# sungnyun/dualhyp

Hardware: AMD Instinct MI355X
Metric: corrected utterances/sec (TinyLlama-1.1B, 5+5 hyps, 512->64 tok) (higher is better)
Workload: dtype bf16; 1 GPU; DualHyp inference, TinyLlama-1.1B bf16 + LoRA r16 (q,k,v,proj), batch 32/GPU synthetic 5+5-hyp prompts, 512-token prompt -> 64 generated tokens, greedy; batch_per_gpu=32, parallelism=replicas x1, batches_in_flight_per_gpu=64, schedule=merged, decode_rows_per_launch=2048

## Files before the change

dualhyp_amd/csrc/capi.hip:

```cpp
#include "common.h"
#include "tuning.h"
#include <stdarg.h>

static thread_local char g_err[512] = "";

void dh_set_error(const char* fmt, ...) {
    va_list ap;
    va_start(ap, fmt);
    vsnprintf(g_err, sizeof(g_err), fmt, ap);
    va_end(ap);
}

extern "C" const char* dh_last_error(void) { return g_err; }
extern "C" int dh_abi_version(void) { return DH_ABI_VERSION; }

extern "C" int dh_device_info(char* h_buf, int h_buf_len, int* h_num_cu, int64_t* h_hbm_bytes) {
    int n = 0;
    hipError_t e = hipGetDeviceCount(&n);
    DH_CHECK(e == hipSuccess && n > 0, "no HIP device visible (%s)", hipGetErrorString(e));
    int dev = 0;
    DH_HIP(hipGetDevice(&dev));
    hipDeviceProp_t p;
    DH_HIP(hipGetDeviceProperties(&p, dev));
    if (h_buf && h_buf_len > 0) {
        strncpy(h_buf, p.gcnArchName, h_buf_len - 1);
        h_buf[h_buf_len - 1] = 0;
    }
    if (h_num_cu) *h_num_cu = p.multiProcessorCount;
    if (h_hbm_bytes) *h_hbm_bytes = (int64_t)p.totalGlobalMem;
    return 0;
}

namespace {

enum Accept { ANY, BOOL , RANGE , ONE_OF  };
struct TuningRow { int key; int* knob; Accept accept; int a, b, c; };
constexpr int NO_MAX = 0x7fffffff;

const TuningRow TUNING[] = {
    {0, &g_skinny_variant, ANY, 0, 0, 0},
    {1, &g_gemm_variant, ANY, 0, 0, 0},
    {2, &g_swiglu2, ANY, 0, 0, 0},
    {3, &g_mid, ANY, 0, 0, 0},
    {4, &g_linear_phase, ANY, 0, 0, 0},
    {5, &g_gemm_gm, RANGE, 0, NO_MAX, 0},
    {6, &g_dt_min_rows, RANGE, 1, NO_MAX, 0},
    {7, &g_chain_min_rows, RANGE, 1, NO_MAX, 0},
    {8, &g_dt_stages, ANY, 0, 0, 0},
    {9, &g_gemm128_stages, ANY, 0, 0, 0},
    {10, &g_decode_tiled_rows, RANGE, 0, NO_MAX, 0},
    {11, &g_rows_ct, RANGE, 0, NO_MAX, 0},
    {12, &g_fuse_qkv_rope, ANY, 0, 0, 0},
    {13, &g_mid_wlds, ANY, 0, 0, 0},
    {14, &g_rows_ng, ONE_OF, 0, 8, 10},
    {15, &g_dt_wide, ANY, 0, 0, 0},
    {16, &g_short_kps, ONE_OF, 8, 16, 16},
    {17, &g_pairs_wn, ONE_OF, 0, 2, 4},
    {18, &g_pairs_min_rows, RANGE, 1, NO_MAX, 0},
    {19, &g_fp8_tile, ONE_OF, 0, 128, 256},
    {20, &g_fp8_gm, RANGE, 0, 64, 0},
    {21, &g_pairs_wt, BOOL, 0, 0, 0},
    {22, &g_w4_persist, RANGE, 0, 2, 0},
    {23, &g_prune_last_layer, BOOL, 0, 0, 0},
    {24, &g_w4_fast_epi, ANY, 0, 0, 0},
    {25, &g_w4_persist_qkv, BOOL, 0, 0, 0},
    {26, &g_tn_mfma, BOOL, 0, 0, 0},
    {27, &g_attn_bwd_dq_group, BOOL, 0, 0, 0},
    {28, &g_tail_split, BOOL, 0, 0, 0},
    {29, &g_attn_bwd_dkdv_img, BOOL, 0, 0, 0},
    {30, &g_w4_persist_lora, BOOL, 0, 0, 0},
    {31, &g_skinny_n, BOOL, 0, 0, 0},
};

}

extern "C" int dh_set_tuning(int key, int value) {
    for (const TuningRow& r : TUNING) {
        if (r.key != key) continue;
        if (r.accept == RANGE && (value < r.a || value > r.b)) break;
        if (r.accept == ONE_OF && value != r.a && value != r.b && value != r.c) break;
        *r.knob = r.accept == BOOL ? value != 0 : value;
        return 0;
    }
    dh_set_error("dh_set_tuning: unknown key %d", key);
    return 1;
}
```

dualhyp_amd/csrc/decode_fused.hip:

```cpp
#include "common.h"

namespace {

constexpr int DCOLS = 16;
constexpr int MAXP = 16;

template <int HS, int PMAX, int NW>
__global__ __launch_bounds__(NW * 64, NW == 16 ? 1 : (NW == 6 ? 3 : (HS == 64 ? 4 : 2))) void attn_decode_fused_kernel(
    const float* __restrict__ qkv32, int n_part, int pairs, int n_seq, int ldq, int qkv_dim,
    const bf16_t* __restrict__ lora_b, float lora_scale, int split0, int split1,
    const bf16_t* __restrict__ cos, const bf16_t* __restrict__ sin, const int32_t* __restrict__ seq_slot,
    const int32_t* __restrict__ kv_len, bf16_t* __restrict__ k_cache, bf16_t* __restrict__ vT_cache,
    bf16_t* __restrict__ y, int n_head, int n_groups, int s_max, float scale) {
    constexpr int KS = HS / 16, DT = HS / 32, HALF = HS / 2;
    extern __shared__ __attribute__((aligned(16))) char smem[];
    const int pair = blockIdx.x, seq = pair / n_groups, g = pair % n_groups;
    const int q_per_kv = n_head / n_groups;
    const int tid = threadIdx.x, lane = tid & 63, wave = tid >> 6;
    const int lr = lane & 31, lh = lane >> 5;
    const int slot = seq_slot[seq];
    const int len = kv_len[seq], pos = len - 1;
    bf16_t* sQ = reinterpret_cast<bf16_t*>(smem);
    float* sKn = reinterpret_cast<float*>(smem + 16 * HS * 2);
    float* sVn = sKn + HS;
    float* sXa = sVn + HS;
    float* sSn = sXa + 48;
    float* sPm = sSn + 16;
    float* sPl = sPm + NW * DCOLS;
    float* sPo = sPl + NW * DCOLS;
    constexpr int NT_ = NW * 64;

    constexpr int PF = NW == 6 ? 2 : 1;
    struct VF { bf16x8 v; };
    struct Tile { bf16x8 kf[KS]; VF vf[DT][2]; };
    Tile tl[PF];
    const bf16_t* kbase = k_cache + ((size_t)slot * n_groups + g) * s_max * HS;
    const bf16_t* vbase = vT_cache + ((size_t)slot * n_groups + g) * HS * s_max;
    const int n_tiles = (pos + 31) / 32;
    auto load_tile = [&](Tile& T, int t) {
#pragma unroll
        for (int ks = 0; ks < KS; ++ks)
            T.kf[ks] = __builtin_nontemporal_load(reinterpret_cast<const bf16x8*>(kbase + kfrag_blk<HS>(t, ks) + lane * 8));
#pragma unroll
        for (int dt = 0; dt < DT; ++dt)
#pragma unroll
            for (int s2 = 0; s2 < 2; ++s2)
                T.vf[dt][s2].v = __builtin_nontemporal_load(reinterpret_cast<const bf16x8*>(vbase + vfrag_blk<HS>(t, dt, s2) + lane * 8));
    };
#pragma unroll
    for (int p = 0; p < PF; ++p)
        if (wave + NW * p < n_tiles) load_tile(tl[p], wave + NW * p);

    const float* row0 = qkv32 + (size_t)seq * ldq;
    const size_t pstride = (size_t)n_seq * ldq;
    auto psum = [&](int c) {
        float v[PMAX];
#pragma unroll
        for (int p = 0; p < PMAX; ++p) v[p] = p < n_part ? row0[p * pstride + c] : 0.f;
        float s = 0.f;
        if (pairs) {
#pragma unroll
            for (int p = 0; p < PMAX; p += 2) s += v[p] + v[p + 1];
        } else {
#pragma unroll
            for (int p = 0; p < PMAX; ++p) s += v[p];
        }
        return s;
    };
    if (lora_b != nullptr && tid < 48) sXa[tid] = rbf(psum(qkv_dim + tid));
    for (int i = tid; i < 16 * HS; i += NT_) sQ[i] = 0;
    __syncthreads();

    auto finish = [&](int c) -> float {
        float o = rbf(psum(c));
        if (lora_b != nullptr) {
            const int seg = (c >= split0) + (c >= split1);
            const uint4* b4 = reinterpret_cast<const uint4*>(lora_b + (size_t)c * 16);
            float l = 0.f;
#pragma unroll
            for (int h = 0; h < 2; ++h) {
                const uint4 bv = b4[h];
                const bf16_t* bp = reinterpret_cast<const bf16_t*>(&bv);
#pragma unroll
                for (int e = 0; e < 8; ++e) l = fmaf(sXa[seg * 16 + h * 8 + e], bf2f(bp[e]), l);
            }
            o = rbf(o + rbf(rbf(l) * lora_scale));
        }
        return o;
    };
    const int gbase = g * (q_per_kv + 2) * HS;
    bf16_t* kdst = k_cache + ((size_t)slot * n_groups + g) * s_max * HS;
    bf16_t* vdst = vT_cache + ((size_t)slot * n_groups + g) * HS * s_max;
    const int n_rope = (q_per_kv + 1) * HALF;
    for (int it = tid; it < n_rope + HS; it += NT_) {
        if (it < n_rope) {
            const int j = it / HALF, i = it % HALF;
            const float x1 = finish(gbase + j * HS + i), x2 = finish(gbase + j * HS + HALF + i);
            const bf16_t* cp = cos + (size_t)pos * HS;
            const bf16_t* sp = sin + (size_t)pos * HS;
            const bf16_t o1 = f2bf(rbf(x1 * bf2f(cp[i])) + rbf(-x2 * bf2f(sp[i])));
            const bf16_t o2 = f2bf(rbf(x2 * bf2f(cp[HALF + i])) + rbf(x1 * bf2f(sp[HALF + i])));
            if (j < q_per_kv) {
                sQ[j * HS + i] = o1;
                sQ[j * HS + HALF + i] = o2;
            } else {
                sKn[i] = bf2f(o1);
                sKn[HALF + i] = bf2f(o2);
                kdst[kfrag_off<HS>(pos, i)] = o1;
                kdst[kfrag_off<HS>(pos, HALF + i)] = o2;
            }
        } else {
            const int e = it - n_rope;
            const bf16_t v = f2bf(finish(gbase + (q_per_kv + 1) * HS + e));
            sVn[e] = bf2f(v);
            vdst[vfrag_off<HS>(pos, e)] = v;
        }
    }
    __syncthreads();

    for (int h = wave; h < q_per_kv; h += NW) {
        float p = 0.f;
        for (int e = lane; e < HS; e += 64) p += bf2f(sQ[h * HS + e]) * sKn[e];
        p = wave_sum(p);
        if (lane == 0) sSn[h] = p * scale;
    }

    bf16x8 qf[KS];
#pragma unroll
    for (int ks = 0; ks < KS; ++ks) qf[ks] = *reinterpret_cast<const bf16x8*>(sQ + (lr & 15) * HS + ks * 16 + lh * 8);
    if (lr >= 16) {
#pragma unroll
        for (int ks = 0; ks < KS; ++ks) qf[ks] = bf16x8{0, 0, 0, 0, 0, 0, 0, 0};
    }
    f32x16 o[DT];
#pragma unroll
    for (int dt = 0; dt < DT; ++dt)
#pragma unroll
        for (int r = 0; r < 16; ++r) o[dt][r] = 0.f;
    float m_run = -INFINITY, l_run = 0.f;
    auto compute_tile = [&](const Tile& T, int t) {
        const int key0 = t * 32;
        f32x16 st;
#pragma unroll
        for (int r = 0; r < 16; ++r) st[r] = 0.f;
#pragma unroll
        for (int ks = 0; ks < KS; ++ks) st = __builtin_amdgcn_mfma_f32_32x32x16_bf16(T.kf[ks], qf[ks], st, 0, 0, 0);
        float m_t = -INFINITY;
#pragma unroll
        for (int r = 0; r < 16; ++r) {
            const int key_abs = key0 + (r & 3) + 8 * (r >> 2) + 4 * lh;
            float sc = st[r] * scale;
            sc = key_abs < pos ? sc : -INFINITY;
            st[r] = sc;
            m_t = fmaxf(m_t, sc);
        }
        m_t = fmaxf(m_t, __shfl_xor(m_t, 32, 64));
        const float m_new = fmaxf(m_run, m_t);
        const float alpha = __expf(m_run - m_new);
        m_run = m_new;
        float psm = 0.f;
#pragma unroll
        for (int r = 0; r < 16; ++r) {
            const float p = __expf(st[r] - m_new);
            st[r] = p;
            psm += p;
        }
        l_run = l_run * alpha + psm;
#pragma unroll
        for (int s2 = 0; s2 < 2; ++s2) {
            union { bf16x8 v; uint32_t u[4]; } pf;
#pragma unroll
            for (int j = 0; j < 4; ++j) pf.u[j] = pack2bf(st[8 * s2 + 2 * j], st[8 * s2 + 2 * j + 1]);
#pragma unroll
            for (int dt = 0; dt < DT; ++dt) {
                if (s2 == 0) {
#pragma unroll
                    for (int r = 0; r < 16; ++r) o[dt][r] *= alpha;
                }
                o[dt] = __builtin_amdgcn_mfma_f32_32x32x16_bf16(T.vf[dt][s2].v, pf.v, o[dt], 0, 0, 0);
            }
        }
    };
    for (int base = wave; base < n_tiles; base += NW * PF) {
#pragma unroll
        for (int p = 0; p < PF; ++p) {
            if (base + NW * p < n_tiles) compute_tile(tl[p], base + NW * p);
            if (base + NW * (PF + p) < n_tiles) load_tile(tl[p], base + NW * (PF + p));
        }
    }
    const float l_tot = l_run + __shfl_xor(l_run, 32, 64);
    if (lr < q_per_kv) {
        if (lh == 0) {
            sPm[wave * DCOLS + lr] = m_run;
            sPl[wave * DCOLS + lr] = l_tot;
        }
#pragma unroll
        for (int dt = 0; dt < DT; ++dt)
#pragma unroll
            for (int r = 0; r < 16; ++r) {
                const int d = dt * 32 + (r & 3) + 8 * (r >> 2) + 4 * lh;
                sPo[(wave * HS + d) * DCOLS + lr] = o[dt][r];
            }
    }
    __syncthreads();
    for (int it = tid; it < q_per_kv * HS; it += NT_) {
        const int h = it / HS, d = it % HS;
        const float sn = sSn[h];
        float M = sn;
#pragma unroll
        for (int w = 0; w < NW; ++w) M = fmaxf(M, sPm[w * DCOLS + h]);
        const float pn = __expf(sn - M);
        float L = pn, O = rbf(pn) * sVn[d];
#pragma unroll
        for (int w = 0; w < NW; ++w) {
            const float mw = sPm[w * DCOLS + h];
            const float f = (mw == -INFINITY) ? 0.f : __expf(mw - M);
            L += sPl[w * DCOLS + h] * f;
            O += sPo[(w * HS + d) * DCOLS + h] * f;
        }
        y[(size_t)seq * n_head * HS + (g * q_per_kv + h) * HS + d] = f2bf(O / L);
    }
}

#ifndef DH_ATTN_WAVES64
#define DH_ATTN_WAVES64 8
#endif
template <int HS>
constexpr int attn_fused_waves() { return HS == 64 ? DH_ATTN_WAVES64 : 8; }
template <int HS>
constexpr size_t attn_fused_lds() {
    constexpr int NW = attn_fused_waves<HS>();
    return 16 * HS * 2 + (HS + HS + 48 + 16 + NW * DCOLS + NW * DCOLS + NW * HS * DCOLS) * sizeof(float);
}

template <int HS, int PMAX, int NW>
__global__ __launch_bounds__(NW * 64, 1) void attn_verify_fused_kernel(
    const float* __restrict__ qkv32, int n_part, int pairs, int n_rows, int ldq, int qkv_dim,
    const bf16_t* __restrict__ lora_b, float lora_scale, int split0, int split1,
    const bf16_t* __restrict__ cos, const bf16_t* __restrict__ sin, const int32_t* __restrict__ seq_slot,
    const int32_t* __restrict__ kv_len, bf16_t* __restrict__ k_cache, bf16_t* __restrict__ vT_cache,
    bf16_t* __restrict__ y, int n_head, int n_groups, int s_max, int p_max, int S, float scale) {
    constexpr int KS = HS / 16, DT = HS / 32, HALF = HS / 2, VC = 32;
    extern __shared__ __attribute__((aligned(16))) char smem[];
    const int pair = blockIdx.x, seq = pair / n_groups, g = pair % n_groups;
    const int q_per_kv = n_head / n_groups, ncol = S * q_per_kv;
    const int tid = threadIdx.x, lane = tid & 63, wave = tid >> 6;
    const int lr = lane & 31, lh = lane >> 5;
    const int slot = seq_slot[seq];
    const int len = kv_len[seq], pos = len - 1;
    const int n_live = min(S, p_max - pos);
    bf16_t* sQ = reinterpret_cast<bf16_t*>(smem);
    float* sKn = reinterpret_cast<float*>(smem + VC * HS * 2);
    float* sVn = sKn + S * HS;
    float* sXa = sVn + S * HS;
    float* sSn = sXa + S * 48;
    float* sPm = sSn + VC;
    float* sPl = sPm + NW * VC;
    float* sPo = sPl + NW * VC;
    constexpr int NT_ = NW * 64;

    struct VF { bf16x8 v; };
    struct Tile { bf16x8 kf[KS]; VF vf[DT][2]; };
    Tile tl;
    const bf16_t* kbase = k_cache + ((size_t)slot * n_groups + g) * s_max * HS;
    const bf16_t* vbase = vT_cache + ((size_t)slot * n_groups + g) * HS * s_max;
    const int n_tiles = (pos + n_live - 1 + 31) / 32;
    const int t_safe = pos >> 5;
    auto load_tile = [&](Tile& T, int t, bool early) {
#pragma unroll
        for (int ks = 0; ks < KS; ++ks) {
            const bf16x8* p = reinterpret_cast<const bf16x8*>(kbase + kfrag_blk<HS>(t, ks) + lane * 8);
            T.kf[ks] = early ? __builtin_nontemporal_load(p) : *p;
        }
#pragma unroll
        for (int dt = 0; dt < DT; ++dt)
#pragma unroll
            for (int s2 = 0; s2 < 2; ++s2) {
                const bf16x8* p = reinterpret_cast<const bf16x8*>(vbase + vfrag_blk<HS>(t, dt, s2) + lane * 8);
                T.vf[dt][s2].v = early ? __builtin_nontemporal_load(p) : *p;
            }
    };
    if (wave < t_safe) load_tile(tl, wave, true);

    const size_t pstride = (size_t)n_rows * ldq;
    auto psum = [&](int j, int c) {
        const float* row0 = qkv32 + ((size_t)seq * S + j) * ldq;
        float v[PMAX];
#pragma unroll
        for (int p = 0; p < PMAX; ++p) v[p] = p < n_part ? row0[p * pstride + c] : 0.f;
        float s = 0.f;
        if (pairs) {
#pragma unroll
            for (int p = 0; p < PMAX; p += 2) s += v[p] + v[p + 1];
        } else {
#pragma unroll
            for (int p = 0; p < PMAX; ++p) s += v[p];
        }
        return s;
    };
    if (lora_b != nullptr)
        for (int i = tid; i < 48 * S; i += NT_) sXa[i] = rbf(psum(i / 48, qkv_dim + i % 48));
    for (int i = tid; i < VC * HS; i += NT_) sQ[i] = 0;
    for (int i = tid; i < 2 * S * HS; i += NT_) sKn[i] = 0.f;
    __syncthreads();

    auto finish = [&](int j, int c) -> float {
        float o = rbf(psum(j, c));
        if (lora_b != nullptr) {
            const int seg = (c >= split0) + (c >= split1);
            const uint4* b4 = reinterpret_cast<const uint4*>(lora_b + (size_t)c * 16);
            float l = 0.f;
#pragma unroll
            for (int h = 0; h < 2; ++h) {
                const uint4 bv = b4[h];
                const bf16_t* bp = reinterpret_cast<const bf16_t*>(&bv);
#pragma unroll
                for (int e = 0; e < 8; ++e) l = fmaf(sXa[j * 48 + seg * 16 + h * 8 + e], bf2f(bp[e]), l);
            }
            o = rbf(o + rbf(rbf(l) * lora_scale));
        }
        return o;
    };
    const int gbase = g * (q_per_kv + 2) * HS;
    bf16_t* kdst = k_cache + ((size_t)slot * n_groups + g) * s_max * HS;
    bf16_t* vdst = vT_cache + ((size_t)slot * n_groups + g) * HS * s_max;
    const int n_rope = (q_per_kv + 1) * HALF, per_row = n_rope + HS;
    for (int it0 = tid; it0 < n_live * per_row; it0 += NT_) {
        const int jr = it0 / per_row, it = it0 % per_row, pj = pos + jr;
        if (it < n_rope) {
            const int j = it / HALF, i = it % HALF;
            const float x1 = finish(jr, gbase + j * HS + i), x2 = finish(jr, gbase + j * HS + HALF + i);
            const bf16_t* cp = cos + (size_t)pj * HS;
            const bf16_t* sp = sin + (size_t)pj * HS;
            const bf16_t o1 = f2bf(rbf(x1 * bf2f(cp[i])) + rbf(-x2 * bf2f(sp[i])));
            const bf16_t o2 = f2bf(rbf(x2 * bf2f(cp[HALF + i])) + rbf(x1 * bf2f(sp[HALF + i])));
            if (j < q_per_kv) {
                sQ[(jr * q_per_kv + j) * HS + i] = o1;
                sQ[(jr * q_per_kv + j) * HS + HALF + i] = o2;
            } else {
                sKn[jr * HS + i] = bf2f(o1);
                sKn[jr * HS + HALF + i] = bf2f(o2);
                kdst[kfrag_off<HS>(pj, i)] = o1;
                kdst[kfrag_off<HS>(pj, HALF + i)] = o2;
            }
        } else {
            const int e = it - n_rope;
            const bf16_t v = f2bf(finish(jr, gbase + (q_per_kv + 1) * HS + e));
            sVn[jr * HS + e] = bf2f(v);
            vdst[vfrag_off<HS>(pj, e)] = v;
        }
    }
    __threadfence_block();
    __syncthreads();
    if (wave >= t_safe && wave < n_tiles) load_tile(tl, wave, false);

    for (int c = wave; c < ncol; c += NW) {
        const float* kn = sKn + (c / q_per_kv) * HS;
        float p = 0.f;
        for (int e = lane; e < HS; e += 64) p += bf2f(sQ[c * HS + e]) * kn[e];
        p = wave_sum(p);
        if (lane == 0) sSn[c] = p * scale;
    }

    bf16x8 qf[KS];
#pragma unroll
    for (int ks = 0; ks < KS; ++ks) qf[ks] = *reinterpret_cast<const bf16x8*>(sQ + lr * HS + ks * 16 + lh * 8);
    const int j_col = lr < ncol ? lr / q_per_kv : 0;
    const int p_col = pos + (j_col < n_live ? j_col : 0);
    f32x16 o[DT];
#pragma unroll
    for (int dt = 0; dt < DT; ++dt)
#pragma unroll
        for (int r = 0; r < 16; ++r) o[dt][r] = 0.f;
    float m_run = -INFINITY, l_run = 0.f;
    auto compute_tile = [&](const Tile& T, int t) {
        const int key0 = t * 32;
        f32x16 st;
#pragma unroll
        for (int r = 0; r < 16; ++r) st[r] = 0.f;
#pragma unroll
        for (int ks = 0; ks < KS; ++ks) st = __builtin_amdgcn_mfma_f32_32x32x16_bf16(T.kf[ks], qf[ks], st, 0, 0, 0);
        float m_t = -INFINITY;
#pragma unroll
        for (int r = 0; r < 16; ++r) {
            const int key_abs = key0 + (r & 3) + 8 * (r >> 2) + 4 * lh;
            float sc = st[r] * scale;
            sc = key_abs < p_col ? sc : -INFINITY;
            st[r] = sc;
            m_t = fmaxf(m_t, sc);
        }
        m_t = fmaxf(m_t, __shfl_xor(m_t, 32, 64));
        const float m_new = fmaxf(m_run, m_t);
        const bool none = m_new == -INFINITY;
        const float alpha = none ? 1.f : __expf(m_run - m_new);
        m_run = m_new;
        float psm = 0.f;
#pragma unroll
        for (int r = 0; r < 16; ++r) {
            const float p = none ? 0.f : __expf(st[r] - m_new);
            st[r] = p;
            psm += p;
        }
        l_run = l_run * alpha + psm;
#pragma unroll
        for (int s2 = 0; s2 < 2; ++s2) {
            union { bf16x8 v; uint32_t u[4]; } pf;
#pragma unroll
            for (int j = 0; j < 4; ++j) pf.u[j] = pack2bf(st[8 * s2 + 2 * j], st[8 * s2 + 2 * j + 1]);
#pragma unroll
            for (int dt = 0; dt < DT; ++dt) {
                if (s2 == 0) {
#pragma unroll
                    for (int r = 0; r < 16; ++r) o[dt][r] *= alpha;
                }
                o[dt] = __builtin_amdgcn_mfma_f32_32x32x16_bf16(T.vf[dt][s2].v, pf.v, o[dt], 0, 0, 0);
            }
        }
    };
    for (int base = wave; base < n_tiles; base += NW) {
        compute_tile(tl, base);
        if (base + NW < n_tiles) load_tile(tl, base + NW, false);
    }
    const float l_tot = l_run + __shfl_xor(l_run, 32, 64);
    if (lr < ncol) {
        if (lh == 0) {
            sPm[wave * VC + lr] = m_run;
            sPl[wave * VC + lr] = l_tot;
        }
#pragma unroll
        for (int dt = 0; dt < DT; ++dt)
#pragma unroll
            for (int r = 0; r < 16; ++r) {
                const int d = dt * 32 + (r & 3) + 8 * (r >> 2) + 4 * lh;
                sPo[(wave * HS + d) * ncol + lr] = o[dt][r];
            }
    }
    __syncthreads();
    for (int it = tid; it < ncol * HS; it += NT_) {
        const int c = it / HS, d = it % HS, jr = c / q_per_kv, h = c % q_per_kv;
        const float sn = sSn[c];
        float M = sn;
#pragma unroll
        for (int w = 0; w < NW; ++w) M = fmaxf(M, sPm[w * VC + c]);
        const float pn = __expf(sn - M);
        float L = pn, O = rbf(pn) * sVn[jr * HS + d];
#pragma unroll
        for (int w = 0; w < NW; ++w) {
            const float mw = sPm[w * VC + c];
            const float f = (mw == -INFINITY) ? 0.f : __expf(mw - M);
            L += sPl[w * VC + c] * f;
            O += sPo[(w * HS + d) * ncol + c] * f;
        }
        y[((size_t)seq * S + jr) * n_head * HS + (g * q_per_kv + h) * HS + d] = f2bf(O / L);
    }
}
template <int HS>
size_t attn_verify_lds(int S, int ncol) {
    constexpr int NW = attn_fused_waves<HS>();
    return 32 * HS * 2 + (size_t)(2 * S * HS + 48 * S + 32 + 2 * NW * 32 + NW * HS * ncol) * sizeof(float);
}

template <int MAXC>
__global__ __launch_bounds__(256) void finish_norm_kernel(const float* __restrict__ h32, int n_part, int pairs, int rows, int ldh,
                                                          const bf16_t* __restrict__ lora_b, float lora_scale,
                                                          const bf16_t* __restrict__ x_resid,
                                                          const bf16_t* __restrict__ w_norm, bf16_t* __restrict__ x_out,
                                                          bf16_t* __restrict__ xn_out, int d, float eps,
                                                          const uint8_t* __restrict__ row_tail) {
    __shared__ float sXa[16];
    __shared__ float sRed[4];
    const int row = blockIdx.x, tid = threadIdx.x, lane = tid & 63, wave = tid >> 6;
    const float* hrow = h32 + (size_t)row * ldh;
    const size_t pstride = (size_t)rows * ldh;
    if (lora_b != nullptr && tid < 16) {
        float pv[MAXP];
#pragma unroll
        for (int p = 0; p < MAXP; ++p) pv[p] = p < n_part ? hrow[p * pstride + d + tid] : 0.f;
        float s = 0.f;
        if (pairs) {
#pragma unroll
            for (int p = 0; p < MAXP; p += 2) s += pv[p] + pv[p + 1];
        } else {
#pragma unroll
            for (int p = 0; p < MAXP; ++p) s += pv[p];
        }
        sXa[tid] = rbf(s);
    }
    __syncthreads();
    float v[MAXC][8];
    float ss = 0.f;
#pragma unroll
    for (int i = 0; i < MAXC; ++i) {
        const int c0 = (tid + i * 256) * 8;
        if (c0 < d) {
            float acc[8];
#pragma unroll
            for (int e = 0; e < 8; ++e) acc[e] = 0.f;
            for (int p0 = 0; p0 < n_part; p0 += 4) {
                float4 a0[4], a1[4];
#pragma unroll
                for (int q = 0; q < 4; ++q) {
                    const int p = p0 + q < n_part ? p0 + q : p0;
                    a0[q] = *reinterpret_cast<const float4*>(hrow + p * pstride + c0);
                    a1[q] = *reinterpret_cast<const float4*>(hrow + p * pstride + c0 + 4);
                }
                if (pairs) {
#pragma unroll
                    for (int q = 0; q < 4; q += 2) {
                        if (p0 + q < n_part) {
                            const bool two = p0 + q + 1 < n_part;
                            const float4 b0 = two ? a0[q + 1] : float4{0.f, 0.f, 0.f, 0.f}, b1 = two ? a1[q + 1] : float4{0.f, 0.f, 0.f, 0.f};
                            acc[0] += a0[q].x + b0.x; acc[1] += a0[q].y + b0.y; acc[2] += a0[q].z + b0.z; acc[3] += a0[q].w + b0.w;
                            acc[4] += a1[q].x + b1.x; acc[5] += a1[q].y + b1.y; acc[6] += a1[q].z + b1.z; acc[7] += a1[q].w + b1.w;
                        }
                    }
                } else {
#pragma unroll
                for (int q = 0; q < 4; ++q) {
                    if (p0 + q < n_part) {
                        acc[0] += a0[q].x; acc[1] += a0[q].y; acc[2] += a0[q].z; acc[3] += a0[q].w;
                        acc[4] += a1[q].x; acc[5] += a1[q].y; acc[6] += a1[q].z; acc[7] += a1[q].w;
                    }
                }
                }
            }
            const uint4 xr = *reinterpret_cast<const uint4*>(x_resid + (size_t)row * d + c0);
            const bf16_t* xp = reinterpret_cast<const bf16_t*>(&xr);
            uint4 xo;
            bf16_t* xop = reinterpret_cast<bf16_t*>(&xo);
#pragma unroll
            for (int e = 0; e < 8; ++e) {
                float o = rbf(acc[e]);
                if (lora_b != nullptr) {
                    const uint4* b4 = reinterpret_cast<const uint4*>(lora_b + (size_t)(c0 + e) * 16);
                    float l = 0.f;
#pragma unroll
                    for (int h = 0; h < 2; ++h) {
                        const uint4 bv = b4[h];
                        const bf16_t* bp = reinterpret_cast<const bf16_t*>(&bv);
#pragma unroll
                        for (int k = 0; k < 8; ++k) l = fmaf(sXa[h * 8 + k], bf2f(bp[k]), l);
                    }
                    o = rbf(o + rbf(rbf(l) * lora_scale));
                }
                xop[e] = f2bf(bf2f(xp[e]) + o);
                v[i][e] = bf2f(xop[e]);
                ss += rbf(v[i][e] * v[i][e]);
            }
            *reinterpret_cast<uint4*>(x_out + (size_t)row * d + c0) = xo;
        }
    }
    ss = wave_sum(ss);
    if (lane == 0) sRed[wave] = ss;
    __syncthreads();
    ss = sRed[0] + sRed[1] + sRed[2] + sRed[3];
    const float ms = rbf(ss / (float)d);
    const float t = rbf(ms + eps);
    const bool tail = row_tail != nullptr && row_tail[row] != 0;
    const float r = tail ? rbf(1.0f / rbf(sqrtf(t))) : rbf(1.0f / sqrtf(t));
#pragma unroll
    for (int i = 0; i < MAXC; ++i) {
        const int c0 = (tid + i * 256) * 8;
        if (c0 < d) {
            const uint4 wu = *reinterpret_cast<const uint4*>(w_norm + c0);
            const bf16_t* wp = reinterpret_cast<const bf16_t*>(&wu);
            uint4 o;
            bf16_t* op = reinterpret_cast<bf16_t*>(&o);
#pragma unroll
            for (int e = 0; e < 8; ++e) op[e] = f2bf(bf2f(wp[e]) * rbf(v[i][e] * r));
            *reinterpret_cast<uint4*>(xn_out + (size_t)row * d + c0) = o;
        }
    }
}

}

extern "C" int dh_attn_decode_fused_bf16(const float* qkv32, int n_part, int pairs, int n_seq, int qkv_dim, int n_ext,
                                         const dh_bf16* lora_b, float lora_scale, int split0, int split1,
                                         const dh_bf16* cos, const dh_bf16* sin, const int32_t* seq_slot,
                                         const int32_t* kv_len, dh_bf16* k_cache, dh_bf16* vT_cache, dh_bf16* y,
                                         int n_head, int n_groups, int hs, int s_max, void* stream) {
    DH_CHECK(qkv32 && cos && sin && seq_slot && kv_len && k_cache && vT_cache && y, "dh_attn_decode_fused_bf16: null argument");
    DH_CHECK(n_groups > 0 && n_head % n_groups == 0 && n_head / n_groups <= DCOLS, "dh_attn_decode_fused_bf16: bad head counts");
    DH_CHECK(hs == 64 || hs == 96 || hs == 128, "dh_attn_decode_fused_bf16: head_size %d unsupported", hs);
    DH_CHECK(s_max % 64 == 0 && n_part >= 1 && n_part <= MAXP, "dh_attn_decode_fused_bf16: bad s_max / n_part");
    DH_CHECK(qkv_dim == (n_head + 2 * n_groups) * hs, "dh_attn_decode_fused_bf16: qkv_dim mismatch");
    DH_CHECK(lora_b == nullptr || n_ext >= 48, "dh_attn_decode_fused_bf16: LoRA needs the 48 x·A^T columns");
    if (n_seq <= 0) return 0;
    const float scale = 1.0f / sqrtf((float)hs);
    hipStream_t s = (hipStream_t)stream;
    dim3 grid(n_seq * n_groups);
#define ATT_LAUNCH(HSV, PM)                                                                                           \
    hipLaunchKernelGGL((attn_decode_fused_kernel<HSV, PM, attn_fused_waves<HSV>()>), grid, dim3(64 * attn_fused_waves<HSV>()), attn_fused_lds<HSV>(), s, qkv32, n_part, pairs, n_seq,  \
                       qkv_dim + n_ext, qkv_dim, lora_b, lora_scale, split0, split1, cos, sin, seq_slot, kv_len, k_cache,  \
                       vT_cache, y, n_head, n_groups, s_max, scale)
    if (hs == 64) {
        DH_MAX_LDS_ONCE((attn_decode_fused_kernel<64, 2, attn_fused_waves<64>()>), attn_fused_lds<64>());
        DH_MAX_LDS_ONCE((attn_decode_fused_kernel<64, 8, attn_fused_waves<64>()>), attn_fused_lds<64>());
        DH_MAX_LDS_ONCE((attn_decode_fused_kernel<64, 16, attn_fused_waves<64>()>), attn_fused_lds<64>());
        if (n_part <= 2) ATT_LAUNCH(64, 2);
        else if (n_part <= 8) ATT_LAUNCH(64, 8);
        else ATT_LAUNCH(64, 16);
    } else if (hs == 96) {
        DH_MAX_LDS_ONCE((attn_decode_fused_kernel<96, 2, 8>), attn_fused_lds<96>());
        DH_MAX_LDS_ONCE((attn_decode_fused_kernel<96, 8, 8>), attn_fused_lds<96>());
        DH_MAX_LDS_ONCE((attn_decode_fused_kernel<96, 16, 8>), attn_fused_lds<96>());
        if (n_part <= 2) ATT_LAUNCH(96, 2);
        else if (n_part <= 8) ATT_LAUNCH(96, 8);
        else ATT_LAUNCH(96, 16);
    } else {
        DH_MAX_LDS_ONCE((attn_decode_fused_kernel<128, 2, 8>), attn_fused_lds<128>());
        DH_MAX_LDS_ONCE((attn_decode_fused_kernel<128, 8, 8>), attn_fused_lds<128>());
        DH_MAX_LDS_ONCE((attn_decode_fused_kernel<128, 16, 8>), attn_fused_lds<128>());
        if (n_part <= 2) ATT_LAUNCH(128, 2);
        else if (n_part <= 8) ATT_LAUNCH(128, 8);
        else ATT_LAUNCH(128, 16);
    }
#undef ATT_LAUNCH
    DH_LAUNCH_CHECK();
    return 0;
}

int dh_attn_verify_fused_impl(const float* qkv32, int n_part, int pairs, int n_seq, int S, int qkv_dim, int n_ext,
                              const dh_bf16* lora_b, float lora_scale, int split0, int split1, const dh_bf16* cos,
                              const dh_bf16* sin, const int32_t* seq_slot, const int32_t* kv_len, dh_bf16* k_cache,
                              dh_bf16* vT_cache, dh_bf16* y, int n_head, int n_groups, int hs, int s_max, int p_max, void* stream) {
    DH_CHECK(qkv32 && cos && sin && seq_slot && kv_len && k_cache && vT_cache && y, "attn_verify_fused: null argument");
    DH_CHECK(n_groups > 0 && n_head % n_groups == 0, "attn_verify_fused: bad head counts");
    DH_CHECK(S >= 2 && S <= 8 && S * (n_head / n_groups) <= 32, "attn_verify_fused: %d positions x %d heads per group exceed 32 query columns",
             S, n_head / n_groups);
    DH_CHECK(hs == 64 || hs == 96 || hs == 128, "attn_verify_fused: head_size %d unsupported", hs);
    DH_CHECK(s_max % 64 == 0 && p_max > 0 && p_max <= s_max && n_part >= 1 && n_part <= MAXP, "attn_verify_fused: bad s_max / p_max / n_part");
    DH_CHECK(qkv_dim == (n_head + 2 * n_groups) * hs, "attn_verify_fused: qkv_dim mismatch");
    DH_CHECK(lora_b == nullptr || n_ext >= 48, "attn_verify_fused: LoRA needs the 48 x·A^T columns");
    if (n_seq <= 0) return 0;
    const float scale = 1.0f / sqrtf((float)hs);
    hipStream_t s = (hipStream_t)stream;
    dim3 grid(n_seq * n_groups);
    const int ncol = S * (n_head / n_groups);
#define VER_LAUNCH(HSV, PM)                                                                                           \
    hipLaunchKernelGGL((attn_verify_fused_kernel<HSV, PM, attn_fused_waves<HSV>()>), grid, dim3(64 * attn_fused_waves<HSV>()), attn_verify_lds<HSV>(S, ncol), s, qkv32, n_part, pairs, \
                       n_seq * S, qkv_dim + n_ext, qkv_dim, lora_b, lora_scale, split0, split1, cos, sin, seq_slot, kv_len, k_cache,  \
                       vT_cache, y, n_head, n_groups, s_max, p_max, S, scale)
#define VER_HS(HSV)                                                                                                   \
    do {                                                                                                              \
        DH_MAX_LDS_ONCE((attn_verify_fused_kernel<HSV, 2, attn_fused_waves<HSV>()>), attn_verify_lds<HSV>(8, 32));    \
        DH_MAX_LDS_ONCE((attn_verify_fused_kernel<HSV, 8, attn_fused_waves<HSV>()>), attn_verify_lds<HSV>(8, 32));    \
        DH_MAX_LDS_ONCE((attn_verify_fused_kernel<HSV, 16, attn_fused_waves<HSV>()>), attn_verify_lds<HSV>(8, 32));   \
        if (n_part <= 2) VER_LAUNCH(HSV, 2);                                                                          \
        else if (n_part <= 8) VER_LAUNCH(HSV, 8);                                                                     \
        else VER_LAUNCH(HSV, 16);                                                                                     \
    } while (0)
    if (hs == 64) VER_HS(64);
    else if (hs == 96) VER_HS(96);
    else VER_HS(128);
#undef VER_HS
#undef VER_LAUNCH
    DH_LAUNCH_CHECK();
    return 0;
}

extern "C" int dh_finish_norm_bf16(const float* h32, int n_part, int pairs, int rows, int d, int n_ext, const dh_bf16* lora_b,
                                   float lora_scale, const dh_bf16* x_resid, const dh_bf16* w_norm, dh_bf16* x_out,
                                   dh_bf16* xn_out, float eps, const uint8_t* row_tail, void* stream) {
    DH_CHECK(h32 && x_resid && w_norm && x_out && xn_out, "dh_finish_norm_bf16: null argument");
    DH_CHECK(d % 8 == 0 && d <= 8192 && n_part >= 1 && n_part <= MAXP, "dh_finish_norm_bf16: unsupported d=%d", d);
    DH_CHECK(lora_b == nullptr || n_ext >= 16, "dh_finish_norm_bf16: LoRA needs the 16 x·A^T columns");
    DH_CHECK((d + n_ext) % 4 == 0, "dh_finish_norm_bf16: row stride must be a multiple of 4 floats");
    if (rows <= 0) return 0;
    hipStream_t s = (hipStream_t)stream;
    dim3 grid(rows), block(256);
    const int ldh = d + n_ext;
#define LAUNCH(MAXC) hipLaunchKernelGGL((finish_norm_kernel<MAXC>), grid, block, 0, s, h32, n_part, pairs, rows, ldh, lora_b, \
                                        lora_scale, x_resid, w_norm, x_out, xn_out, d, eps, row_tail)
    if (d <= 2048) { LAUNCH(1); }
    else if (d <= 4096) { LAUNCH(2); }
    else { LAUNCH(4); }
#undef LAUNCH
    DH_LAUNCH_CHECK();
    return 0;
}
```

dualhyp_amd/csrc/tuning.h:

```cpp
#pragma once

extern int g_gemm128_stages, g_gemm_variant, g_tail_split, g_linear_phase;
extern int g_gemm_gm, g_w4_persist, g_w4_fast_epi, g_w4_persist_qkv, g_w4_persist_lora;
extern int g_mid, g_mid_wlds;
extern int g_dt_stages, g_dt_wide, g_dt_min_rows, g_chain_min_rows, g_pairs_wn, g_pairs_wt;
extern int g_pairs_min_rows, g_skinny_n;
__attribute__((visibility("hidden"))) extern int g_skinny_variant, g_swiglu2, g_rows_ct, g_rows_ng;
extern int g_fp8_tile, g_fp8_gm;
extern int g_decode_tiled_rows, g_short_kps, g_fuse_qkv_rope, g_prune_last_layer;
extern int g_attn_bwd_dkdv_img, g_attn_bwd_dq_group;
extern int g_tn_mfma;
```

Measured before the change: 804.9 utterances/s.

## Add latency-chained decode attention kernel and hoist finish-norm loads

```diff
diff --git a/dualhyp_amd/csrc/capi.hip b/dualhyp_amd/csrc/capi.hip
--- a/dualhyp_amd/csrc/capi.hip
+++ b/dualhyp_amd/csrc/capi.hip
@@ -70,6 +70,8 @@
     {29, &g_attn_bwd_dkdv_img, BOOL, 0, 0, 0},
     {30, &g_w4_persist_lora, BOOL, 0, 0, 0},
     {31, &g_skinny_n, BOOL, 0, 0, 0},
+    {40, &g_attn_chain, BOOL, 0, 0, 0},
+    {41, &g_finish_hoist_rows, RANGE, -1, NO_MAX, 0},
 };
 
 }
diff --git a/dualhyp_amd/csrc/decode_fused.hip b/dualhyp_amd/csrc/decode_fused.hip
--- a/dualhyp_amd/csrc/decode_fused.hip
+++ b/dualhyp_amd/csrc/decode_fused.hip
@@ -1,4 +1,20 @@
 #include "common.h"
+#include "tuning.h"
+
+int g_attn_chain = 1;
+int g_finish_hoist_rows = -1;
+
+#ifdef DH_ATTN_STAMPS
+__device__ unsigned long long g_attn_stamps[4096 * 8];
+#define ATTN_STAMP(i) do { if (threadIdx.x == 0 && blockIdx.x < 4096) g_attn_stamps[blockIdx.x * 8 + (i)] = __builtin_amdgcn_s_memrealtime(); } while (0)
+#define ATTN_DRAIN() __builtin_amdgcn_s_waitcnt(0)
+extern "C" int dh_debug_attn_stamps(unsigned long long* out) {
+    return hipMemcpyFromSymbol(out, HIP_SYMBOL(g_attn_stamps), sizeof(g_attn_stamps)) == hipSuccess ? 0 : 1;
+}
+#else
+#define ATTN_STAMP(i)
+#define ATTN_DRAIN()
+#endif
 
 namespace {
 
@@ -29,6 +45,7 @@
     float* sPl = sPm + NW * DCOLS;
     float* sPo = sPl + NW * DCOLS;
     constexpr int NT_ = NW * 64;
+    ATTN_STAMP(0);
 
     constexpr int PF = NW == 6 ? 2 : 1;
     struct VF { bf16x8 v; };
@@ -70,6 +87,7 @@
     if (lora_b != nullptr && tid < 48) sXa[tid] = rbf(psum(qkv_dim + tid));
     for (int i = tid; i < 16 * HS; i += NT_) sQ[i] = 0;
     __syncthreads();
+    ATTN_STAMP(1);
 
     auto finish = [&](int c) -> float {
         float o = rbf(psum(c));
@@ -117,6 +135,7 @@
         }
     }
     __syncthreads();
+    ATTN_STAMP(2);
 
     for (int h = wave; h < q_per_kv; h += NW) {
         float p = 0.f;
@@ -187,7 +206,14 @@
             if (base + NW * p < n_tiles) compute_tile(tl[p], base + NW * p);
             if (base + NW * (PF + p) < n_tiles) load_tile(tl[p], base + NW * (PF + p));
         }
-    }
+#ifdef DH_ATTN_STAMPS
+        if (base == wave) { asm volatile("" :: "v"(o[0][0])); ATTN_STAMP(3); }
+#endif
+    }
+#ifdef DH_ATTN_STAMPS
+    asm volatile("" :: "v"(o[0][0]));
+#endif
+    ATTN_STAMP(4);
     const float l_tot = l_run + __shfl_xor(l_run, 32, 64);
     if (lr < q_per_kv) {
         if (lh == 0) {
@@ -203,6 +229,7 @@
             }
     }
     __syncthreads();
+    ATTN_STAMP(5);
     for (int it = tid; it < q_per_kv * HS; it += NT_) {
         const int h = it / HS, d = it % HS;
         const float sn = sSn[h];
@@ -220,6 +247,9 @@
         }
         y[(size_t)seq * n_head * HS + (g * q_per_kv + h) * HS + d] = f2bf(O / L);
     }
+    ATTN_STAMP(6);
+    ATTN_DRAIN();
+    ATTN_STAMP(7);
 }
 
 #ifndef DH_ATTN_WAVES64
@@ -231,6 +261,256 @@
 constexpr size_t attn_fused_lds() {
     constexpr int NW = attn_fused_waves<HS>();
     return 16 * HS * 2 + (HS + HS + 48 + 16 + NW * DCOLS + NW * DCOLS + NW * HS * DCOLS) * sizeof(float);
+}
+
+constexpr int CHAIN_NW = 8;
+template <int HS>
+constexpr size_t attn_chain_lds() {
+    return 16 * HS * 2 + (HS + HS + 48 + 16 + CHAIN_NW * DCOLS + CHAIN_NW * DCOLS + CHAIN_NW * DCOLS * (HS + 8)) * sizeof(float);
+}
+
+template <int HS, int PMAX, int NW>
+__global__ __launch_bounds__(NW * 64, HS == 64 ? 4 : 2) void attn_decode_chain_kernel(
+    const float* __restrict__ qkv32, int n_part, int pairs, int n_seq, int ldq, int qkv_dim,
+    const bf16_t* __restrict__ lora_b, float lora_scale, int split0, int split1,
+    const bf16_t* __restrict__ cos, const bf16_t* __restrict__ sin, const int32_t* __restrict__ seq_slot,
+    const int32_t* __restrict__ kv_len, bf16_t* __restrict__ k_cache, bf16_t* __restrict__ vT_cache,
+    bf16_t* __restrict__ y, int n_head, int n_groups, int s_max, float scale) {
+    static_assert(NW == CHAIN_NW, "one tile in flight per wave and the occupancy asked for above are those of the 8-wave form");
+    constexpr int KS = HS / 16, DT = HS / 32, HALF = HS / 2;
+    extern __shared__ __attribute__((aligned(16))) char smem[];
+    const int pair = blockIdx.x, seq = pair / n_groups, g = pair % n_groups;
+    const int q_per_kv = n_head / n_groups;
+    const int tid = threadIdx.x, lane = tid & 63, wave = tid >> 6;
+    const int lr = lane & 31, lh = lane >> 5;
+    bf16_t* sQ = reinterpret_cast<bf16_t*>(smem);
+    float* sKn = reinterpret_cast<float*>(smem + 16 * HS * 2);
+    float* sVn = sKn + HS;
+    float* sXa = sVn + HS;
+    float* sSn = sXa + 48;
+    float* sPm = sSn + 16;
+    float* sPl = sPm + NW * DCOLS;
+    float* sPo = sPl + NW * DCOLS;
+    constexpr int PST = HS + 8;
+    constexpr int NT_ = NW * 64;
+    ATTN_STAMP(0);
+
+    const int slot = seq_slot[seq];
+    const int len = kv_len[seq], pos = len - 1;
+
+    const float* row0 = qkv32 + (size_t)seq * ldq;
+    const size_t pstride = (size_t)n_seq * ldq;
+    auto pload = [&](int c, float (&v)[PMAX]) {
+#pragma unroll
+        for (int p = 0; p < PMAX; ++p) v[p] = p < n_part ? row0[p * pstride + c] : 0.f;
+    };
+    auto padd = [&](const float (&v)[PMAX]) {
+        float s = 0.f;
+        if (pairs) {
+#pragma unroll
+            for (int p = 0; p < PMAX; p += 2) s += v[p] + v[p + 1];
+        } else {
+#pragma unroll
+            for (int p = 0; p < PMAX; ++p) s += v[p];
+        }
+        return s;
+    };
+    const int gbase = g * (q_per_kv + 2) * HS;
+    const int n_rope = (q_per_kv + 1) * HALF;
+    const bool is_rope = tid < n_rope, is_val = !is_rope && tid < n_rope + HS;
+    const int rj = tid / HALF, ri = tid % HALF, ve = tid - n_rope;
+    const int c1 = is_rope ? gbase + rj * HS + ri : (is_val ? gbase + (q_per_kv + 1) * HS + ve : gbase);
+    const int c2 = is_rope ? c1 + HALF : gbase;
+    const bool has_xa = lora_b != nullptr && tid < 48;
+    float vx[PMAX], v1[PMAX], v2[PMAX];
+    uint4 b1[2], b2[2];
+    pload(has_xa ? qkv_dim + tid : 0, vx);
+    pload(c1, v1);
+    pload(c2, v2);
+    if (lora_b != nullptr) {
+        const uint4* b4 = reinterpret_cast<const uint4*>(lora_b + (size_t)c1 * 16);
+        b1[0] = b4[0]; b1[1] = b4[1];
+        b4 = reinterpret_cast<const uint4*>(lora_b + (size_t)c2 * 16);
+        b2[0] = b4[0]; b2[1] = b4[1];
+    } else {
+        b1[0] = b1[1] = b2[0] = b2[1] = uint4{0, 0, 0, 0};
+    }
+    const bf16_t* cp = cos + (size_t)pos * HS;
+    const bf16_t* sp = sin + (size_t)pos * HS;
+    const bf16_t cs[4] = {cp[ri], sp[ri], cp[HALF + ri], sp[HALF + ri]};
+
+    struct VF { bf16x8 v; };
+    struct Tile { bf16x8 kf[KS]; VF vf[DT][2]; };
+    Tile tl;
+    const bf16_t* kbase = k_cache + ((size_t)slot * n_groups + g) * s_max * HS;
+    const bf16_t* vbase = vT_cache + ((size_t)slot * n_groups + g) * HS * s_max;
+    const int n_tiles = (pos + 31) / 32;
+    auto load_tile = [&](Tile& T, int t) {
+#pragma unroll
+        for (int ks = 0; ks < KS; ++ks)
+            T.kf[ks] = __builtin_nontemporal_load(reinterpret_cast<const bf16x8*>(kbase + kfrag_blk<HS>(t, ks) + lane * 8));
+#pragma unroll
+        for (int dt = 0; dt < DT; ++dt)
+#pragma unroll
+            for (int s2 = 0; s2 < 2; ++s2)
+                T.vf[dt][s2].v = __builtin_nontemporal_load(reinterpret_cast<const bf16x8*>(vbase + vfrag_blk<HS>(t, dt, s2) + lane * 8));
+    };
+    load_tile(tl, wave < n_tiles ? wave : (n_tiles > 0 ? n_tiles - 1 : 0));
+
+    if (has_xa) sXa[tid] = rbf(padd(vx));
+    __syncthreads();
+    ATTN_STAMP(1);
+
+    auto finish = [&](const float (&v)[PMAX], int c, const uint4 (&b)[2]) -> float {
+        float o = rbf(padd(v));
+        if (lora_b != nullptr) {
+            const int seg = (c >= split0) + (c >= split1);
+            float l = 0.f;
+#pragma unroll
+            for (int h = 0; h < 2; ++h) {
+                const uint4 bv = b[h];
+                const bf16_t* bp = reinterpret_cast<const bf16_t*>(&bv);
+#pragma unroll
+                for (int e = 0; e < 8; ++e) l = fmaf(sXa[seg * 16 + h * 8 + e], bf2f(bp[e]), l);
+            }
+            o = rbf(o + rbf(rbf(l) * lora_scale));
+        }
+        return o;
+    };
+    bf16_t* kdst = k_cache + ((size_t)slot * n_groups + g) * s_max * HS;
+    bf16_t* vdst = vT_cache + ((size_t)slot * n_groups + g) * HS * s_max;
+    if (is_rope) {
+        const int j = rj, i = ri;
+        const float x1 = finish(v1, c1, b1), x2 = finish(v2, c2, b2);
+        const bf16_t o1 = f2bf(rbf(x1 * bf2f(cs[0])) + rbf(-x2 * bf2f(cs[1])));
+        const bf16_t o2 = f2bf(rbf(x2 * bf2f(cs[2])) + rbf(x1 * bf2f(cs[3])));
+        if (j < q_per_kv) {
+            sQ[j * HS + i] = o1;
+            sQ[j * HS + HALF + i] = o2;
+        } else {
+            sKn[i] = bf2f(o1);
+            sKn[HALF + i] = bf2f(o2);
+            kdst[kfrag_off<HS>(pos, i)] = o1;
+            kdst[kfrag_off<HS>(pos, HALF + i)] = o2;
+        }
+    } else if (is_val) {
+        const bf16_t v = f2bf(finish(v1, c1, b1));
+        sVn[ve] = bf2f(v);
+        vdst[vfrag_off<HS>(pos, ve)] = v;
+    }
+    __syncthreads();
+    ATTN_STAMP(2);
+
+    for (int h = wave; h < q_per_kv; h += NW) {
+        float p = 0.f;
+        for (int e = lane; e < HS; e += 64) p += bf2f(sQ[h * HS + e]) * sKn[e];
+        p = wave_sum(p);
+        if (lane == 0) sSn[h] = p * scale;
+    }
+
+    bf16x8 qf[KS];
+#pragma unroll
+    for (int ks = 0; ks < KS; ++ks) qf[ks] = *reinterpret_cast<const bf16x8*>(sQ + (lr & 15) * HS + ks * 16 + lh * 8);
+    if (lr >= q_per_kv) {
+#pragma unroll
+        for (int ks = 0; ks < KS; ++ks) qf[ks] = bf16x8{0, 0, 0, 0, 0, 0, 0, 0};
+    }
+    f32x16 o[DT];
+#pragma unroll
+    for (int dt = 0; dt < DT; ++dt)
+#pragma unroll
+        for (int r = 0; r < 16; ++r) o[dt][r] = 0.f;
+    float m_run = -INFINITY, l_run = 0.f;
+    auto compute_tile = [&](const Tile& T, int t) {
+        const int key0 = t * 32;
+        f32x16 st;
+#pragma unroll
+        for (int r = 0; r < 16; ++r) st[r] = 0.f;
+#pragma unroll
+        for (int ks = 0; ks < KS; ++ks) st = __builtin_amdgcn_mfma_f32_32x32x16_bf16(T.kf[ks], qf[ks], st, 0, 0, 0);
+        float m_t = -INFINITY;
+#pragma unroll
+        for (int r = 0; r < 16; ++r) {
+            const int key_abs = key0 + (r & 3) + 8 * (r >> 2) + 4 * lh;
+            float sc = st[r] * scale;
+            sc = key_abs < pos ? sc : -INFINITY;
+            st[r] = sc;
+            m_t = fmaxf(m_t, sc);
+        }
+        m_t = fmaxf(m_t, __shfl_xor(m_t, 32, 64));
+        const float m_new = fmaxf(m_run, m_t);
+        const float alpha = __expf(m_run - m_new);
+        m_run = m_new;
+        float psm = 0.f;
+#pragma unroll
+        for (int r = 0; r < 16; ++r) {
+            const float p = __expf(st[r] - m_new);
+            st[r] = p;
+            psm += p;
+        }
+        l_run = l_run * alpha + psm;
+#pragma unroll
+        for (int s2 = 0; s2 < 2; ++s2) {
+            union { bf16x8 v; uint32_t u[4]; } pf;
+#pragma unroll
+            for (int j = 0; j < 4; ++j) pf.u[j] = pack2bf(st[8 * s2 + 2 * j], st[8 * s2 + 2 * j + 1]);
+#pragma unroll
+            for (int dt = 0; dt < DT; ++dt) {
+                if (s2 == 0) {
+#pragma unroll
+                    for (int r = 0; r < 16; ++r) o[dt][r] *= alpha;
+                }
+                o[dt] = __builtin_amdgcn_mfma_f32_32x32x16_bf16(T.vf[dt][s2].v, pf.v, o[dt], 0, 0, 0);
+            }
+        }
+    };
+    for (int base = wave; base < n_tiles; base += NW) {
+        compute_tile(tl, base);
+        if (base + NW < n_tiles) load_tile(tl, base + NW);
+#ifdef DH_ATTN_STAMPS
+        if (base == wave) { asm volatile("" :: "v"(o[0][0])); ATTN_STAMP(3); }
+#endif
+    }
+#ifdef DH_ATTN_STAMPS
+    asm volatile("" :: "v"(o[0][0]));
+#endif
+    ATTN_STAMP(4);
+    const float l_tot = l_run + __shfl_xor(l_run, 32, 64);
+    if (lr < q_per_kv) {
+        if (lh == 0) {
+            sPm[wave * DCOLS + lr] = m_run;
+            sPl[wave * DCOLS + lr] = l_tot;
+        }
+#pragma unroll
+        for (int dt = 0; dt < DT; ++dt)
+#pragma unroll
+            for (int r = 0; r < 16; ++r) {
+                const int d = dt * 32 + (r & 3) + 8 * (r >> 2) + 4 * lh;
+                sPo[(wave * DCOLS + lr) * PST + d] = o[dt][r];
+            }
+    }
+    __syncthreads();
+    ATTN_STAMP(5);
+    for (int it = tid; it < q_per_kv * HS; it += NT_) {
+        const int h = it / HS, d = it % HS;
+        const float sn = sSn[h];
+        float M = sn;
+#pragma unroll
+        for (int w = 0; w < NW; ++w) M = fmaxf(M, sPm[w * DCOLS + h]);
+        const float pn = __expf(sn - M);
+        float L = pn, O = rbf(pn) * sVn[d];
+#pragma unroll
+        for (int w = 0; w < NW; ++w) {
+            const float mw = sPm[w * DCOLS + h];
+            const float f = (mw == -INFINITY) ? 0.f : __expf(mw - M);
+            L += sPl[w * DCOLS + h] * f;
+            O += sPo[(w * DCOLS + h) * PST + d] * f;
+        }
+        y[(size_t)seq * n_head * HS + (g * q_per_kv + h) * HS + d] = f2bf(O / L);
+    }
+    ATTN_STAMP(6);
+    ATTN_DRAIN();
+    ATTN_STAMP(7);
 }
 
 template <int HS, int PMAX, int NW>
@@ -460,7 +740,7 @@
     return 32 * HS * 2 + (size_t)(2 * S * HS + 48 * S + 32 + 2 * NW * 32 + NW * HS * ncol) * sizeof(float);
 }
 
-template <int MAXC>
+template <int MAXC, bool HOIST>
 __global__ __launch_bounds__(256) void finish_norm_kernel(const float* __restrict__ h32, int n_part, int pairs, int rows, int ldh,
                                                           const bf16_t* __restrict__ lora_b, float lora_scale,
                                                           const bf16_t* __restrict__ x_resid,
@@ -486,6 +766,19 @@
         }
         sXa[tid] = rbf(s);
     }
+    float4 ha0[4] = {}, ha1[4] = {};
+    uint4 hxr = {}, hwu = {};
+    if (HOIST && tid * 8 < d) {
+        const int c0 = tid * 8;
+#pragma unroll
+        for (int q = 0; q < 4; ++q) {
+            const int p = q < n_part ? q : 0;
+            ha0[q] = *reinterpret_cast<const float4*>(hrow + p * pstride + c0);
+            ha1[q] = *reinterpret_cast<const float4*>(hrow + p * pstride + c0 + 4);
+        }
+        hxr = *reinterpret_cast<const uint4*>(x_resid + (size_t)row * d + c0);
+        hwu = *reinterpret_cast<const uint4*>(w_norm + c0);
+    }
     __syncthreads();
     float v[MAXC][8];
     float ss = 0.f;
@@ -500,6 +793,10 @@
                 float4 a0[4], a1[4];
 #pragma unroll
                 for (int q = 0; q < 4; ++q) {
+                    if (HOIST && i == 0 && p0 == 0) {
+                        a0[q] = ha0[q]; a1[q] = ha1[q];
+                        continue;
+                    }
                     const int p = p0 + q < n_part ? p0 + q : p0;
                     a0[q] = *reinterpret_cast<const float4*>(hrow + p * pstride + c0);
                     a1[q] = *reinterpret_cast<const float4*>(hrow + p * pstride + c0 + 4);
@@ -524,7 +821,7 @@
                 }
                 }
             }
-            const uint4 xr = *reinterpret_cast<const uint4*>(x_resid + (size_t)row * d + c0);
+            const uint4 xr = HOIST && i == 0 ? hxr : *reinterpret_cast<const uint4*>(x_resid + (size_t)row * d + c0);
             const bf16_t* xp = reinterpret_cast<const bf16_t*>(&xr);
             uint4 xo;
             bf16_t* xop = reinterpret_cast<bf16_t*>(&xo);
@@ -562,7 +859,7 @@
     for (int i = 0; i < MAXC; ++i) {
         const int c0 = (tid + i * 256) * 8;
         if (c0 < d) {
-            const uint4 wu = *reinterpret_cast<const uint4*>(w_norm + c0);
+            const uint4 wu = HOIST && i == 0 ? hwu : *reinterpret_cast<const uint4*>(w_norm + c0);
             const bf16_t* wp = reinterpret_cast<const bf16_t*>(&wu);
             uint4 o;
             bf16_t* op = reinterpret_cast<bf16_t*>(&o);
@@ -594,11 +891,23 @@
     hipLaunchKernelGGL((attn_decode_fused_kernel<HSV, PM, attn_fused_waves<HSV>()>), grid, dim3(64 * attn_fused_waves<HSV>()), attn_fused_lds<HSV>(), s, qkv32, n_part, pairs, n_seq,  \
                        qkv_dim + n_ext, qkv_dim, lora_b, lora_scale, split0, split1, cos, sin, seq_slot, kv_len, k_cache,  \
                        vT_cache, y, n_head, n_groups, s_max, scale)
+#define CHAIN_LAUNCH(PM)                                                                                              \
+    hipLaunchKernelGGL((attn_decode_chain_kernel<64, PM, CHAIN_NW>), grid, dim3(64 * CHAIN_NW), attn_chain_lds<64>(), s, qkv32, n_part, pairs, n_seq,  \
+                       qkv_dim + n_ext, qkv_dim, lora_b, lora_scale, split0, split1, cos, sin, seq_slot, kv_len, k_cache,  \
+                       vT_cache, y, n_head, n_groups, s_max, scale)
     if (hs == 64) {
         DH_MAX_LDS_ONCE((attn_decode_fused_kernel<64, 2, attn_fused_waves<64>()>), attn_fused_lds<64>());
         DH_MAX_LDS_ONCE((attn_decode_fused_kernel<64, 8, attn_fused_waves<64>()>), attn_fused_lds<64>());
         DH_MAX_LDS_ONCE((attn_decode_fused_kernel<64, 16, attn_fused_waves<64>()>), attn_fused_lds<64>());
-        if (n_part <= 2) ATT_LAUNCH(64, 2);
+        const bool chain = g_attn_chain != 0 && attn_fused_waves<64>() == CHAIN_NW && (n_head / n_groups + 1) * 32 + 64 <= 64 * CHAIN_NW;
+        if (chain) {
+            DH_MAX_LDS_ONCE((attn_decode_chain_kernel<64, 2, CHAIN_NW>), attn_chain_lds<64>());
+            DH_MAX_LDS_ONCE((attn_decode_chain_kernel<64, 8, CHAIN_NW>), attn_chain_lds<64>());
+            DH_MAX_LDS_ONCE((attn_decode_chain_kernel<64, 16, CHAIN_NW>), attn_chain_lds<64>());
+            if (n_part <= 2) CHAIN_LAUNCH(2);
+            else if (n_part <= 8) CHAIN_LAUNCH(8);
+            else CHAIN_LAUNCH(16);
+        } else if (n_part <= 2) ATT_LAUNCH(64, 2);
         else if (n_part <= 8) ATT_LAUNCH(64, 8);
         else ATT_LAUNCH(64, 16);
     } else if (hs == 96) {
@@ -617,6 +926,7 @@
         else ATT_LAUNCH(128, 16);
     }
 #undef ATT_LAUNCH
+#undef CHAIN_LAUNCH
     DH_LAUNCH_CHECK();
     return 0;
 }
@@ -660,6 +970,8 @@
     return 0;
 }
 
+constexpr int FINISH_HOIST_ROWS = 128;
+
 extern "C" int dh_finish_norm_bf16(const float* h32, int n_part, int pairs, int rows, int d, int n_ext, const dh_bf16* lora_b,
                                    float lora_scale, const dh_bf16* x_resid, const dh_bf16* w_norm, dh_bf16* x_out,
                                    dh_bf16* xn_out, float eps, const uint8_t* row_tail, void* stream) {
@@ -671,8 +983,14 @@
     hipStream_t s = (hipStream_t)stream;
     dim3 grid(rows), block(256);
     const int ldh = d + n_ext;
-#define LAUNCH(MAXC) hipLaunchKernelGGL((finish_norm_kernel<MAXC>), grid, block, 0, s, h32, n_part, pairs, rows, ldh, lora_b, \
-                                        lora_scale, x_resid, w_norm, x_out, xn_out, d, eps, row_tail)
+#define LAUNCH(MAXC) do {                                                                                             \
+        if (hoist) hipLaunchKernelGGL((finish_norm_kernel<MAXC, true>), grid, block, 0, s, h32, n_part, pairs, rows, ldh, lora_b,  \
+                                      lora_scale, x_resid, w_norm, x_out, xn_out, d, eps, row_tail);                  \
+        else hipLaunchKernelGGL((finish_norm_kernel<MAXC, false>), grid, block, 0, s, h32, n_part, pairs, rows, ldh, lora_b,       \
+                                lora_scale, x_resid, w_norm, x_out, xn_out, d, eps, row_tail);                        \
+    } while (0)
+    const int hoist_rows = g_finish_hoist_rows >= 0 ? g_finish_hoist_rows : FINISH_HOIST_ROWS;
+    const bool hoist = hoist_rows > 0 && rows >= hoist_rows;
     if (d <= 2048) { LAUNCH(1); }
     else if (d <= 4096) { LAUNCH(2); }
     else { LAUNCH(4); }
diff --git a/dualhyp_amd/csrc/tuning.h b/dualhyp_amd/csrc/tuning.h
--- a/dualhyp_amd/csrc/tuning.h
+++ b/dualhyp_amd/csrc/tuning.h
@@ -10,3 +10,4 @@
 extern int g_decode_tiled_rows, g_short_kps, g_fuse_qkv_rope, g_prune_last_layer;
 extern int g_attn_bwd_dkdv_img, g_attn_bwd_dq_group;
 extern int g_tn_mfma;
+extern int g_attn_chain, g_finish_hoist_rows;
```

Measured after the change: 819.9 utterances/s, median of 6. 1.9% higher.
